# akshathmangudi/KAN-ViT

Measured on AMD Instinct MI355X. Metric: images/sec (train step) KAN-ViT 224x224, higher is better.
Workload: dtype f32

## Files before the change

kan-vit_amd/csrc/kan_bwd_weight_dma.hip:

```cpp
#include "kan_layer_common.h"

namespace {

typedef const __attribute__((address_space(1))) void* kvd_glb_ptr;
typedef __attribute__((address_space(3))) void* kvd_lds_ptr;

#ifndef KVD_NSLOT_N
#define KVD_NSLOT_N 4
#endif
constexpr int KVD_NSLOT = KVD_NSLOT_N;
constexpr int KVD_BLK = 16;
#ifndef KVD_ABLATE
#define KVD_ABLATE 0
#endif

template <int N>
__device__ __forceinline__ void kvd_wait_vm() {
    asm volatile("s_waitcnt vmcnt(%0)" ::"n"(N) : "memory");
}

template <int FAM, int GP, int NOT, bool BF>
__global__ __launch_bounds__(256) void kan_bwd_weight_dma_kernel(const LayerArgs a, int nfb, int nos, int tiles_per_bg, int shared,
                                                                 int nbg, int sub_rows, int cap, int placed) {
    constexpr int XF = KVD_BLK * 32;
    constexpr int YW = 32 * NOT;
    constexpr int SLOTF = XF + KVD_BLK * YW;
    constexpr int NDX = XF / 256;
    constexpr int NDY = KVD_BLK * YW / 256;
    constexpr int NDMA = NDX + NDY;
    static_assert(XF % 256 == 0 && (KVD_BLK * YW) % 256 == 0, "whole DMA instructions");
    static_assert(NDMA * (KVD_NSLOT - 1) < 64, "vmcnt is a 6-bit counter");
    extern __shared__ __attribute__((aligned(16))) float smem[];
    const int lane = threadIdx.x & 63, l31 = lane & 31, hf = lane >> 5;
    const int wave = __builtin_amdgcn_readfirstlane(threadIdx.x >> 6);
    const int gsz = nfb * nos;
    const int L = (int)(blockIdx.x & 7) * cap + (int)(blockIdx.x >> 3);
    int bg, slab, fb, os;
    if (placed) {
        const int set = L / gsz, mem = L - set * gsz;
        if (set >= nbg * a.msplit) return;
        bg = set % nbg, slab = set / nbg;
        fb = mem % nfb, os = mem / nfb;
    } else {
        const int units = gsz * nbg;
        if (L >= units * a.msplit) return;
        const int u = L % units;
// ... 33 lines not shown
    const char* dybase = reinterpret_cast<const char*>(a.dy + ms * a.ldy);
    int xrow[NDX], xcol[NDX], yrow[NDY], ycol[NDY];
#pragma unroll
    for (int k = 0; k < NDX; ++k) {
        const int c = 64 * k + lane;
        xrow[k] = c >> 3;
        xcol[k] = (c & 7) * 4;
    }
#pragma unroll
    for (int k = 0; k < NDY; ++k) {
        const int c = 64 * k + lane;
        const int row = c / (8 * NOT), rem = c - row * (8 * NOT), tile = rem >> 3;
        int tc = tcol[0];
#pragma unroll
        for (int i = 1; i < NOT; ++i) tc = tile == i ? tcol[i] : tc;
        yrow[k] = row;
        ycol[k] = tc + (rem & 7) * 4;
    }
    unsigned xo[NDX], yo[NDY];
#pragma unroll
    for (int k = 0; k < NDX; ++k) xo[k] = 4u * (unsigned)(xrow[k] * ldx32 + xcol[k]);
#pragma unroll
    for (int k = 0; k < NDY; ++k) yo[k] = 4u * (unsigned)(yrow[k] * ldy32 + ycol[k]);
    float* ring = smem + wave * (KVD_NSLOT * SLOTF);

    auto issue = [&](int blk, int slot) __attribute__((always_inline)) {
        if (KVD_ABLATE & 2) return;
        float* dst = ring + slot * SLOTF;
        const bool ragged = (blk + 1) * KVD_BLK > len;
        if (!ragged) {
            const char* xb = xbase + (long long)blk * (KVD_BLK * 4) * ldx32;
            const char* yb = dybase + (long long)blk * (KVD_BLK * 4) * ldy32;
#pragma unroll
            for (int k = 0; k < NDX; ++k) __builtin_amdgcn_global_load_lds((kvd_glb_ptr)(xb + xo[k]), (kvd_lds_ptr)(dst + 256 * k), 16, 0, 0);
#pragma unroll
            for (int k = 0; k < NDY; ++k) __builtin_amdgcn_global_load_lds((kvd_glb_ptr)(yb + yo[k]), (kvd_lds_ptr)(dst + XF + 256 * k), 16, 0, 0);
        } else {
#pragma unroll
            for (int k = 0; k < NDX; ++k) {
                int r = blk * KVD_BLK + xrow[k];
                r = r < len ? r : len - 1;
                __builtin_amdgcn_global_load_lds((kvd_glb_ptr)(xbase + 4u * (unsigned)(r * ldx32 + xcol[k])), (kvd_lds_ptr)(dst + 256 * k), 16, 0, 0);
            }
#pragma unroll
            for (int k = 0; k < NDY; ++k) {
                int r = blk * KVD_BLK + yrow[k];
                r = r < len ? r : len - 1;
                __builtin_amdgcn_global_load_lds((kvd_glb_ptr)(dybase + 4u * (unsigned)(r * ldy32 + ycol[k])), (kvd_lds_ptr)(dst + XF + 256 * k), 16, 0, 0);
            }
        }
    };

    constexpr int G0 = (FAM == KV_CHEBY && !BF) ? 1 : 0;
// ... 144 lines not shown
    __syncthreads();
    if (wave != 0) return;
    img = smem + lane;
    add();

    float* base = a.slab + (long long)slab * ((long long)a.groups * a.K * a.O);
#pragma unroll
    for (int i = 0; i < NOT; ++i) {
        if (tg[i] < 0) continue;
        const int tt = os * NOT + i;
        const int col0 = (tt % otpg) * 32;
        float* gb = base + (long long)tg[i] * a.K * a.O + col0 + l31;
#pragma unroll
        for (int j = 0; j < GP; ++j)
#pragma unroll
            for (int r = 0; r < 16; ++r) {
                const int fr = fb * 32 + kv_acc_row(r, hf);
                gb[((long long)fr * GP + j) * a.O] = j < G0 ? csum[i] : acc[j - G0][i][r];
            }
    }
}

template <int FAM, int GP, int NOT, bool BF>
int launch_dma(LayerArgs& a, const LayerBwdWeightPlan& pl, hipStream_t st) {
    const BwRegPlan& p = pl.r;
    const long long gsz = (long long)p.nfb * p.nos, sets = (long long)p.nbg * pl.slabs;
    const long long per_xcd = (sets * gsz + 7) / 8;
    const int placed = gsz <= 32 ? 1 : 0;
    const long long cap = placed ? (per_xcd + gsz - 1) / gsz * gsz : per_xcd;
    dim3 grid((unsigned)(8 * cap), 1, 1);
    constexpr size_t lds = sizeof(float) * 4 * KVD_NSLOT * (KVD_BLK * 32 * (1 + NOT));
    KV_ALLOW_LDS(160 * 1024, (kan_bwd_weight_dma_kernel<FAM, GP, NOT, BF>));
    hipLaunchKernelGGL((kan_bwd_weight_dma_kernel<FAM, GP, NOT, BF>), grid, dim3(256), lds, st, a, p.nfb, p.nos, p.tiles_per_bg, p.shared, p.nbg,
                       (int)(pl.rows_per_slab / 4), (int)cap, placed);
    KV_LAUNCH_CHECK("kan_bwd_weight_dma_kernel");
    return 0;
}

}

int kv_bwd_weight_dma(LayerArgs& a, const LayerBwdWeightPlan& p, hipStream_t st) {
    return p.bf ? launch_dma<KV_CHEBY, 5, 3, true>(a, p, st) : launch_dma<KV_CHEBY, 5, 3, false>(a, p, st);
}
```

kan-vit_amd/csrc/kan_bwd_weight_reg.hip:

```cpp
#include "kan_layer_common.h"

namespace {

template <int N, int I = 0, typename F>
__device__ __forceinline__ void kv_static_for(F&& f) {
    if constexpr (I < N) {
        f(std::integral_constant<int, I>{});
        kv_static_for<N, I + 1>(f);
    }
}

template <int FAM, int GP, int NOT, bool BF, int JC, bool PG, int ACT>
__device__ __forceinline__ void kan_bwd_weight_reg_kbody(const LayerArgs& a, int nfb, int nos, int tiles_per_bg, int shared, int nbg) {
    static_assert(!(PG && FAM == KV_RBF), "FastKAN's patch embedding reads u = LayerNorm(x): no gather form");
    static_assert(!(PG && BF), "the gather form is exact fp32 (bf16 MFMA phases are too short to hide the row walker: launch_bwd_weight_reg)");
    constexpr int NJC = (GP + JC - 1) / JC;
    constexpr bool RBF = (FAM == KV_RBF);
    constexpr int TS = BF ? 8 : 1;
    constexpr int UB = BF ? 1 : 4;
    constexpr int PD = BF ? (GP >= 28 ? 2 : 3) : 2;
    constexpr int NTOK = TS * UB;
    constexpr bool SCALAR_WAVE = FAM == KV_BSPLINE || FAM == KV_RBF || GP >= 28 || PG;
    const int lane = threadIdx.x & 63, l31 = lane & 31, hf = lane >> 5;
    const int wave = SCALAR_WAVE ? __builtin_amdgcn_readfirstlane(threadIdx.x >> 6) : (int)(threadIdx.x >> 6);
// ... 531 lines not shown
int kv_bwd_weight_reg(int family, LayerArgs& a, const LayerBwdWeightPlan& p, hipStream_t st) {
    if (p.form == LAYER_BWW_REG16) {
        if (family == KANVIT_RBF) return launch_bwd_weight_reg16<KV_RBF, 9, 9, 4>(a, p, st);
        return p.r.nt == 12 ? launch_bwd_weight_reg16<KV_BSPLINE, 9, 3, 12>(a, p, st) : launch_bwd_weight_reg16<KV_BSPLINE, 9, 3, 4>(a, p, st);
    }
    switch (family) {
        case KANVIT_LINEAR: return launch_bwd_weight_reg<KV_LINEAR, 1, 6>(a, p, st);
        case KANVIT_CHEBY: return p.r.nt == 1 ? launch_bwd_weight_reg<KV_CHEBY, 5, 1>(a, p, st) : launch_bwd_weight_reg<KV_CHEBY, 5, 3>(a, p, st);
        case KANVIT_BSPLINE:
            return p.r.nt == 3 ? launch_bwd_weight_reg<KV_BSPLINE, 9, 3, 5>(a, p, st) : launch_bwd_weight_reg<KV_BSPLINE, 9, 2, 5>(a, p, st);
        case KANVIT_RBF: return launch_bwd_weight_reg<KV_RBF, 9, 2>(a, p, st);
        case KANVIT_SINE:
            if (a.flags & KANVIT_FLAG_SINE_DFREQ) {
                if (a.GP == 28) return launch_bwd_weight_reg<KV_SINE_DF, 28, 4, 4>(a, p, st);
                return a.GP == 4 ? launch_bwd_weight_reg<KV_SINE_DF, 4, 2>(a, p, st) : launch_bwd_weight_reg<KV_SINE_DF, 5, 2>(a, p, st);
            }
            if (a.GP == 28) return launch_bwd_weight_reg<KV_SINE, 28, 4, 4>(a, p, st);
            return a.GP == 4 ? launch_bwd_weight_reg<KV_SINE, 4, 2>(a, p, st) : launch_bwd_weight_reg<KV_SINE, 5, 2>(a, p, st);
        case KANVIT_FOURIER: return launch_bwd_weight_reg<KV_FOURIER, 56, 4, 4>(a, p, st);
        default: return kv_fail(KANVIT_EINVAL, "unknown family %d", family);
    }
}

BwRegPlan plan_bwd_weight_reg(const kanvit_layer_desc* d) {
    BwRegPlan p{};
    if (kv_config().no_reg || kv_config().no_reg_bw) return p;
    p.njc = 1;
    p.gp = gp_of(d);
    const int fam = d->family;
    const RegBasis* rb = kv_reg_basis(d);
    if (!rb) return p;
    if (fam == KANVIT_BSPLINE && (d->flags & KANVIT_FLAG_BF16_MFMA) && !kv_config().no_bf16 && kv_config().bs_bw_bf16 == 1) return p;
    p.nt = rb->bww_nt;
    p.njc = rb->bww_njc;
    if (d->I % 32 || d->O % 32 || d->M < 256) return p;
    const int nshare = d->groups / d->x_group_mod;
    bool bf16_mode = (d->flags & KANVIT_FLAG_BF16_MFMA) && !kv_config().no_bf16;
    if (fam == KANVIT_BSPLINE && bf16_mode && kv_config().bs_bw_bf16 == 2) bf16_mode = false;
    p.bf = bf16_mode ? 1 : 0;
    if (((fam == KANVIT_BSPLINE && p.njc == 2) || fam == KANVIT_RBF) && !bf16_mode && !kv_config().bw_no_t16) {
        const int sh = (kv_share_ok(fam, d->flags) && nshare > 1) ? 1 : 0;
        const int t16 = (sh ? nshare : 1) * (d->O / 16);
        const int nc = (fam != KANVIT_RBF && t16 % 12 == 0) ? 12 : ((t16 % 4 == 0) ? 4 : 0);
        if (nc) {
            p.t16 = 1;
            p.shared = sh;
            p.nbg = sh ? d->x_group_mod : d->groups;
// ... 13 lines not shown
            if (S < 1) S = 1;
            if (S > 65535) return BwRegPlan{};
            long long rps = (d->M + S - 1) / S;
            rps = (rps + 15) / 16 * 16;
            p.rows_per_slab = rps;
            p.slabs = (int)((d->M + rps - 1) / rps);
            long long ld = d->ldx > d->ldy ? d->ldx : d->ldy;
            if (d->ldu > ld) ld = d->ldu;
            if (rps * ld + ld >= (1LL << 29) || units > (1LL << 30)) return BwRegPlan{};
            p.ok = true;
            return p;
        }
    }
    p.shared = (kv_share_ok(fam, d->flags) && nshare > 1) ? 1 : 0;
    p.nbg = p.shared ? d->x_group_mod : d->groups;
    p.tiles_per_bg = (p.shared ? nshare : 1) * (d->O / 32);
    p.nfb = d->I / 32;
    if (fam == KANVIT_BSPLINE && p.tiles_per_bg <= 2) p.nt = 2;
    p.nos = (p.tiles_per_bg + p.nt - 1) / p.nt;
    if (fam == KANVIT_CHEBY && p.nt == 3 && (long long)p.nbg * p.nfb * p.nos * (d->M / 64) < 4LL * N_CU && !kv_config().bw_dma_force) {
        p.nt = 1;
        p.nos = p.tiles_per_bg;
    }
    if (fam == KANVIT_CHEBY && p.nt == 3 && !kv_config().bw_no_dma && (bf16_mode || d->groups > 1) && d->ldx % 4 == 0 && d->ldy % 4 == 0) {
        const long long units = (long long)p.nbg * p.nfb * p.nos;
        long long r = 1;
        while ((long long)N_CU * r < units) ++r;
        long long S = (long long)N_CU * r / units;
        const bool force = kv_config().bw_dma_force != 0;
        const long long smax = force ? (d->M / 64 > 0 ? d->M / 64 : 1) : d->M / 256;
        if (S > smax) S = smax;
        if (S >= 1 && S <= 65535 && (force || units * S * 100 >= 85LL * N_CU * r)) {
            long long rps = (d->M + S - 1) / S;
            rps = (rps + 63) / 64 * 64;
            const long long ld = d->ldx > d->ldy ? d->ldx : d->ldy;
            if (rps / 4 * ld + ld < (1LL << 29) && units * S < (1LL << 31)) {
                p.dma = 1;
                p.rows_per_slab = rps;
                p.slabs = (int)((d->M + rps - 1) / rps);
                p.ok = true;
                return p;
            }
        }
    }
    const long long units = (long long)p.nbg * p.nfb * p.nos * p.njc;
    long long r = 1;
    while (4LL * N_CU * r < units) ++r;
    long long S = 4LL * N_CU * r / units;
    const long long smax = d->M / 64;
    if (S > smax) S = smax;
    if (S < 1) S = 1;
    if (S > 65535) S = 65535;
    const bool ln = fam == KANVIT_RBF && (d->flags & KANVIT_FLAG_FUSED_LN);
    if (ln && S * 4096 < d->M) S = (d->M + 4095) / 4096;
// ... 24 lines not shown
```

kan-vit_amd/csrc/kan_fwd_reg.hip:

```cpp
#include "kan_layer_common.h"

namespace {

template <int FAM, int NT, int NSH, int ICH, int GPC, int ACT>
__device__ __forceinline__ void kan_fwd_reg_body(const LayerArgs& a, float* __restrict__ smem, const int bx, const int by) {
    constexpr int BN = 32 * NT;
    constexpr int WROW = NSH * BN;
    constexpr int V4 = BN / 4;
    constexpr int IC = 2 * ICH;
    constexpr bool RBF = (FAM == KV_RBF);
    const int tid = threadIdx.x, lane = tid & 63, wave = tid >> 6, l31 = lane & 31, hf = lane >> 5;
    const int ntn = a.O / BN;
    const int gs = bx / ntn;
    const int n0 = (bx - gs * ntn) * BN;
    const int nsets = a.groups / NSH;
    const long long m0 = (long long)by * BM;
    constexpr int G0 = (FAM == KV_CHEBY && GPC > 0) ? 1 : 0;
    const int GP = GPC > 0 ? GPC : a.GP, GPE = GP - G0, KC = IC * GPE;
    const int nch = a.I / IC;
    const int WSZ = KC * WROW;
    const int mrem = (m0 + BM <= a.M) ? BM : (int)(a.M - m0);
    float* W_s = smem;

    const BasisArgs b = make_basis(a, gs);
// ... 238 lines not shown
            float* yp = a.y + yrow * a.ldy + (long long)g * a.O + col;
            const float* bp = a.bias ? a.bias + (long long)g * a.O + col : nullptr;
#pragma unroll
            for (int q = 0; q < 4; ++q) {
                f32x4 v = {acc[t][4 * q], acc[t][4 * q + 1], acc[t][4 * q + 2], acc[t][4 * q + 3]};
                if constexpr (G0 > 0) v += *reinterpret_cast<const f32x4*>(b_s + t * 32 + 8 * q + 4 * hf);
                if (bp) v += *reinterpret_cast<const f32x4*>(bp + 8 * q);
                if (posrow) v += *reinterpret_cast<const f32x4*>(posrow + col + 8 * q);
                *reinterpret_cast<f32x4*>(yp + 8 * q) = v;
                if (cls_owner) {
                    f32x4 cv = *reinterpret_cast<const f32x4*>(a.cls + col + 8 * q);
                    if (a.pos) cv += *reinterpret_cast<const f32x4*>(a.pos + col + 8 * q);
                    *reinterpret_cast<f32x4*>(yp - a.ldy + 8 * q) = cv;
                }
            }
        }
    }
}

template <int FAM, int NT, int NSH, int ICH, int GPC, bool TAIL, int ACT>
__device__ __forceinline__ void kan_fwd_reg_kbody(const LayerArgs& a) {
    extern __shared__ __attribute__((aligned(16))) float smem[];
    if constexpr (TAIL) {
        static_assert(NSH == 3, "the tail hands single projections of a shared-basis launch to the NSH = 1 body");
        const int ty = (int)blockIdx.y - a.tail_y0;
        if (ty >= 0) {
            const int tile = ty / 3, proj = ty - 3 * tile;
            kan_fwd_reg_body<FAM, NT, 1, ICH, GPC, ACT>(a, smem, proj * (int)gridDim.x + (int)blockIdx.x, a.tail_y0 + tile);
            return;
        }
    }
    kan_fwd_reg_body<FAM, NT, NSH, ICH, GPC, ACT>(a, smem, (int)blockIdx.x, (int)blockIdx.y);
}
template <int FAM, int NT, int NSH, int ICH, int GPC = 0, bool TAIL = false>
__global__ __launch_bounds__(256, GPC ? 2 : 1) void kan_fwd_reg_kernel(const LayerArgs a) {
    kan_fwd_reg_kbody<FAM, NT, NSH, ICH, GPC, TAIL, KV_ACT_SILU>(a);
}
template <int FAM, int NT, int NSH, int ICH, int GPC = 0, bool TAIL = false>
__global__ __launch_bounds__(256, GPC ? 2 : 1) void kan_fwd_reg_act_kernel(const LayerArgs a) {
    kan_fwd_reg_kbody<FAM, NT, NSH, ICH, GPC, TAIL, KV_ACT_DYN>(a);
}

template <int FAM, int NT, int NSH, int ICH, int GPC = 0>
int launch_fwd_reg(const LayerArgs& a, const LayerFwdPlan& p, hipStream_t st) {
    const dim3 grid(p.gx, p.gy, 1);
    if constexpr (NSH == 3 && GPC > 0) {
        if (p.tail_y0 != 0x7fffffff) {
            KV_ACT_ALLOW_LDS(FAM, a.base_act, 160 * 1024, kan_fwd_reg_kernel, kan_fwd_reg_act_kernel, (FAM, NT, NSH, ICH, GPC, true));
            KV_ACT_LAUNCH(FAM, a.base_act, kan_fwd_reg_kernel, kan_fwd_reg_act_kernel, (FAM, NT, NSH, ICH, GPC, true), grid, dim3(256), p.lds, st, a);
            KV_LAUNCH_CHECK("kan_fwd_reg_kernel");
            return 0;
        }
    }
    KV_ACT_ALLOW_LDS(FAM, a.base_act, 160 * 1024, kan_fwd_reg_kernel, kan_fwd_reg_act_kernel, (FAM, NT, NSH, ICH, GPC));
    KV_ACT_LAUNCH(FAM, a.base_act, kan_fwd_reg_kernel, kan_fwd_reg_act_kernel, (FAM, NT, NSH, ICH, GPC), grid, dim3(256), p.lds, st, a);
    KV_LAUNCH_CHECK("kan_fwd_reg_kernel");
    return 0;
}

template <int FAM, int NT, int NSH>
int launch_fwd_reg_ich(const LayerArgs& a, const LayerFwdPlan& p, hipStream_t st) {
    if (p.gpc && p.ich == 4) {
        if constexpr (FAM == KV_LINEAR) return launch_fwd_reg<FAM, NT, NSH, 4, 1>(a, p, st);
        if constexpr (FAM == KV_CHEBY) return launch_fwd_reg<FAM, NT, NSH, 4, 5>(a, p, st);
        if constexpr (FAM == KV_BSPLINE || FAM == KV_RBF) return launch_fwd_reg<FAM, NT, NSH, 4, 9>(a, p, st);
        if constexpr (FAM == KV_SINE) return launch_fwd_reg<FAM, NT, NSH, 4, 4>(a, p, st);
    }
    if (p.gpc && p.ich == 2) {
        if constexpr (FAM == KV_BSPLINE || FAM == KV_RBF) return launch_fwd_reg<FAM, NT, NSH, 2, 9>(a, p, st);
// ... 32 lines not shown
```

kan-vit_amd/csrc/kan_layer.hip:

```cpp
#include "kan_layer_common.h"

extern "C" int kanvit_layer_ln_fusable(const kanvit_layer_desc* d);

namespace {

int validate(const kanvit_layer_desc* d, const char* who) {
    if (!d) return kv_fail(KANVIT_EINVAL, "%s: null descriptor", who);
    const int gp = gp_of(d);
    if (gp < 1) return kv_fail(KANVIT_EINVAL, "%s: unknown family %d or G=%d", who, d->family, d->G);
    if (gp > 80) return kv_fail(KANVIT_EINVAL, "%s: %d generated columns per feature exceeds the supported 80", who, gp);
    if (d->groups < 1 || d->x_group_mod < 1 || d->groups % d->x_group_mod != 0)
        return kv_fail(KANVIT_EINVAL, "%s: groups=%d must be a positive multiple of x_group_mod=%d", who, d->groups,
                       d->x_group_mod);
    if (d->groups > 65535) return kv_fail(KANVIT_EINVAL, "%s: groups=%d exceeds 65535", who, d->groups);
    if ((d->M + BM - 1) / BM > 65535) return kv_fail(KANVIT_EINVAL, "%s: M=%lld exceeds %d rows per launch", who,
                                                     (long long)d->M, 65535 * BM);
    if (d->I < 1 || d->O < 1 || d->M < 0) return kv_fail(KANVIT_EINVAL, "%s: bad sizes M=%lld I=%d O=%d", who,
                                                          (long long)d->M, d->I, d->O);
    if ((long long)d->I * gp > 0x7fffffffLL / 4) return kv_fail(KANVIT_EINVAL, "%s: K too large", who);
    if (d->ldx < (int64_t)d->x_group_mod * d->I) return kv_fail(KANVIT_EINVAL, "%s: ldx=%lld < x_group_mod*I", who,
                                                                 (long long)d->ldx);
    if (d->ldy < (int64_t)d->groups * d->O) return kv_fail(KANVIT_EINVAL, "%s: ldy=%lld < groups*O", who,
                                                            (long long)d->ldy);
    if (d->family == KANVIT_BSPLINE) {
        const int nk = d->G + d->spline_order + 1;
        if (d->spline_order < 0 || d->G < 1 || nk > KV_MAX_KNOTS)
            return kv_fail(KANVIT_EINVAL, "%s: bspline G=%d order=%d unsupported (knots %d > %d)", who, d->G,
// ... 84 lines not shown
    if (fam == KANVIT_SINE && ((al.bp & 15) || (d->bparam_stride & 3))) return;
    const long long ldx = pd ? d->I : d->ldx;
    const bool has_u = fam == KANVIT_RBF && al.has_u && !is_ln(d);
    const int wrow = 32 * nt * nsh, wrs = 256 / (8 * nt);
    const RegBasis* rb = kv_config().no_pipe ? nullptr : kv_reg_basis(d);
    for (int ich = 4; ich >= 1; ich >>= 1) {
        const int ic = 2 * ich, kc = ic * gp;
        if (d->I % ic) continue;
        if (pd && (((pd->W / pd->n_patches) % ic) || (ich == 4 && (pd->W & 3)))) continue;
        if (ich == 4 && ((ldx & 3) || (d->I & 3) || (al.x & 15) || (has_u && ((d->ldu & 3) || (al.u & 15))))) continue;
        if ((kc + wrs - 1) / wrs > (share3 ? 4 : 8)) continue;
        if ((long long)kc * d->O >= (1LL << 30)) continue;
        size_t lds = sizeof(float) * 2 * (size_t)kc * wrow;
        if (lds < sizeof(float) * 4 * 32 * 36) lds = sizeof(float) * 4 * 32 * 36;
        if (lds > 160 * 1024) continue;
        p.form = LAYER_FWD_REG;
        p.nt = nt;
        p.nsh = nsh;
        p.ich = ich;
        p.gpc = rb ? rb->fwd_gpc[ich == 4 ? 0 : (ich == 2 ? 1 : 2)] : 0;
        p.lds = lds;
        p.gx = (unsigned)((d->groups / nsh) * (d->O / (32 * nt)));
        p.gy = (unsigned)tiles;
        if (nsh == 3 && p.gpc > 0) {
            const int t1 = kv_tail_first_tile(tiles, (int)p.gx);
            if (t1 < tiles) {
                p.tail_y0 = t1;
                p.gy = (unsigned)(t1 + 3 * (tiles - t1));
            }
        }
        return;
    }
}

void plan_fwd_reg_bf16_form(const kanvit_layer_desc* d, const kanvit_patch_desc* pd, LayerFwdPlan& p) {
    const FwdRegBf16Plan& r = p.rb;
    p.nt = r.nt;
    p.nsh = r.nsh;
    p.ich = r.ich;
    p.ws_bytes = r.ws_bytes;
    p.gx = (unsigned)((d->groups / r.nsh) * (d->O / (32 * r.nt)));
    p.gy = (unsigned)((d->M + BM - 1) / BM);
    p.lds = r.lds;
    p.form = pd ? LAYER_FWD_REG_BF16_PATCH : LAYER_FWD_REG_BF16;
    if (pd || r.ich != 8 || !(d->family == KANVIT_LINEAR || d->family == KANVIT_CHEBY)) return;
    const size_t wlds = (size_t)r.nch * r.vs * 2 * 32 * r.nt * r.nsh * 16 + sizeof(float) * 32 * r.nt * r.nsh;
    if (wlds > 150 * 1024 || r.nch != 4 || d->M < 4096 || p.gx > N_CU || kv_config().no_ws) return;
    const long long ntiles = (d->M + KV_WS_THREADS / 2 - 1) / (KV_WS_THREADS / 2);
    long long py = N_CU / p.gx;
    if (py > ntiles) py = ntiles;
    if (py < 1) py = 1;
// ... 147 lines not shown
                p.nci = d->I / ic;
                p.lds = sizeof(float) * (2 * 16 * ws2 + (fam == KANVIT_SINE ? (size_t)nshare * 4 * gp : 0));
                if (fam != KANVIT_SINE && p.nci > 1) p.tail_y0 = kv_tail_first_tile(tiles, d->x_group_mod);
                const long long t1 = p.tail_y0 < tiles ? p.tail_y0 : tiles;
                p.gy = (unsigned)(t1 + p.nci * (tiles - t1));
                return p;
            }
        }
        if (is_ln(d)) return plan_none(p, "kanvit_layer_bwd_input: KANVIT_FLAG_FUSED_LN needs the register kernel (alignment / shape)");
        p.form = LAYER_BWI_TILE;
        p.ic = kv_tile_bwd_input_ic(fam, d->I, gp, d->G, nshare, 0);
        if (!p.ic) return plan_none(p, "kanvit_layer_bwd_input: tile does not fit the LDS");
    }
    p.kt = (p.ic * gp + 31) / 32;
    p.nci = (d->I + p.ic - 1) / p.ic;
    p.lds = kv_tile_bwd_input_lds(fam, p.ic, gp, d->G, nshare, p.form == LAYER_BWI_TILE_BF16 ? d->O : 0);
    return p;
}

static const char* const KV_PATCH_BWW_UNCOVERED =
    "kanvit_patch_embed_bwd_weight: layer / geometry not covered by the gathering weight-gradient kernels "
    "(kanvit_patch_embed_bwd_weight_ok); use patchify + kanvit_layer_bwd_weight";

LayerBwdWeightPlan plan_layer_bwd_weight(const kanvit_layer_desc* d, const kanvit_patch_desc* pd, const LayerAlign& al) {
    LayerBwdWeightPlan p{};
    p.total = (long long)d->groups * d->I * gp_of(d) * d->O;
    auto slabs = [&p](int ws_slabs, int n, long long rows) {
        p.slabs = n;
        p.rows_per_slab = rows;
        p.ws_bytes = ws_slabs > 1 ? sizeof(float) * (size_t)ws_slabs * (size_t)p.total : 0;
    };
    if (kv_tiny_ok(d)) {
        if (pd) return plan_none(p, KV_PATCH_BWW_UNCOVERED);
        const int s = (int)((d->M + 127) / 128 < 64 ? (d->M + 127) / 128 : 64);
        const long long rows = ((d->M + s - 1) / s + 63) / 64 * 64;
        slabs(s, (int)((d->M + rows - 1) / rows), rows);
        p.form = LAYER_BWW_TINY;
        return p;
    }
    p.r = plan_bwd_weight_reg(d);
    if (p.r.ok) {
        slabs(p.r.slabs, p.r.slabs, p.r.rows_per_slab);
        p.bf = p.r.bf;
        if (pd) {
            if (d->groups != 1 || p.r.bf || p.r.t16 || !kv_reg_basis(d)->bww_pg) return plan_none(p, KV_PATCH_BWW_UNCOVERED);
            p.form = LAYER_BWW_REG_PATCH;
        } else if (p.r.t16) {
            p.form = LAYER_BWW_REG16;
        } else {
            p.form = (p.r.dma && !((al.x | al.dy) & 15)) ? LAYER_BWW_DMA : LAYER_BWW_REG;
        }
        return p;
    }
    if (pd) return plan_none(p, KV_PATCH_BWW_UNCOVERED);
    p.t = plan_bwd_weight(d);
    slabs(p.t.msplit, p.t.msplit, p.t.rows_per_split);
    p.bf = ((d->flags & KANVIT_FLAG_BF16_MFMA) && !kv_config().no_bf16) ? 1 : 0;
    if (is_ln(d)) return plan_none(p, "kanvit_layer_bwd_weight: KANVIT_FLAG_FUSED_LN needs the register kernel (shape)");
    if ((long long)BW_ROWS * d->ldy >= (1LL << 30)) return plan_none(p, "kanvit_layer_bwd_weight: ldy too large for 32-bit tile offsets");
    const int kt = (p.t.ic * gp_of(d) + 31) / 32;
    p.lds = sizeof(float) * 2 * ((size_t)BW_ROWS * (p.t.ic | 1) * (d->family == KANVIT_RBF ? 2 : 1) + (size_t)BW_ROWS * 32 * BW_NT * p.t.nsh +
                                 (size_t)kt * 32 * BW_AS);
    if (p.lds > 160 * 1024) return plan_none(p, "kanvit_layer_bwd_weight: tile does not fit the LDS");
    p.form = p.bf ? LAYER_BWW_TILE_BF16 : LAYER_BWW_TILE;
    return p;
}

static KvTinyArgs tiny_args(const kanvit_layer_desc* d) {
    KvTinyArgs t{};
// ... 181 lines not shown
    patch_args(a, p, cls, pos);
    const LayerFwdPlan pl = plan_layer_fwd(d, p, layer_align(images, nullptr, w, bparams ? bparams : w, bias ? bias : w, y, nullptr, nullptr, nullptr));
    return launch_layer_fwd(d, a, pl, "kanvit_patch_embed_fwd", workspace, workspace_bytes, (hipStream_t)stream);
}

int kanvit_patch_embed_fwd(const kanvit_layer_desc* d, const kanvit_patch_desc* p, const float* images, const float* w,
                           const float* bparams, const float* bias, const float* cls, const float* pos, float* y, void* stream) {
    if (d && (d->flags & KANVIT_FLAG_BF16_MFMA) && !kv_config().no_bf16)
        return kv_fail(KANVIT_EINVAL, "kanvit_patch_embed_fwd: KANVIT_FLAG_BF16_MFMA needs a workspace (kanvit_patch_embed_fwd_ws)");
    return kanvit_patch_embed_fwd_ws(d, p, images, w, bparams, bias, cls, pos, y, nullptr, 0, stream);
}

static bool patch_bwd_weight_geometry_ok(const kanvit_layer_desc* d, const kanvit_patch_desc* p) {
    if (!desc_ok(d) || !p || d->groups != 1 || d->x_group_mod != 1 || d->M < 1) return false;
    if (p->C < 1 || p->H < 1 || p->W < 1 || p->n_patches < 1 || p->H % p->n_patches || p->W % p->n_patches) return false;
    if (p->prepend_rows != 0 && p->prepend_rows != 1) return false;
    const long long P = (long long)p->n_patches * p->n_patches;
    if (d->I != (long long)p->C * (p->H / p->n_patches) * (p->W / p->n_patches) || d->M % P) return false;
    const long long B = d->M / P;
    return B * p->C * p->H * p->W < (1LL << 31) && (d->M + B * p->prepend_rows + 1) * d->ldy < (1LL << 31);
}

int kanvit_patch_embed_bwd_weight_ok(const kanvit_layer_desc* d, const kanvit_patch_desc* p) {
    return patch_bwd_weight_geometry_ok(d, p) && plan_layer_bwd_weight(d, p, LayerAlign{}).form == LAYER_BWW_REG_PATCH;
}

size_t kanvit_patch_embed_bwd_weight_workspace(const kanvit_layer_desc* d, const kanvit_patch_desc* p) {
    if (!patch_bwd_weight_geometry_ok(d, p)) return 0;
    const LayerBwdWeightPlan pl = plan_layer_bwd_weight(d, p, LayerAlign{});
    return pl.form == LAYER_BWW_REG_PATCH ? pl.ws_bytes : 0;
}

static int launch_layer_bwd_weight(const kanvit_layer_desc* d, LayerArgs& a, const LayerBwdWeightPlan& p, float* dw, void* workspace,
                                   hipStream_t st) {
    if (p.form == LAYER_BWW_NONE) return kv_fail(KANVIT_EINVAL, p.why, p.why_a, p.why_b);
    a.rows_per_split = p.rows_per_slab;
    a.msplit = p.slabs;
    a.slab = p.slabs > 1 ? (float*)workspace : dw;
    int rc;
    switch (p.form) {
        case LAYER_BWW_TINY: {
            KvTinyArgs t = tiny_args(d);
            t.x = a.x; t.bp = a.bp; t.dy = a.dy;
            t.slabs = p.slabs; t.rows_per_slab = p.rows_per_slab; t.slab = a.slab;
            rc = kv_tiny_bwd_weight(t, st);
            break;
        }
        case LAYER_BWW_DMA: rc = kv_bwd_weight_dma(a, p, st); break;
        case LAYER_BWW_REG16:
        case LAYER_BWW_REG:
        case LAYER_BWW_REG_PATCH: rc = kv_bwd_weight_reg(d->family, a, p, st); break;
        default:
            a.IC = p.t.ic;
            a.nchunks_n = p.t.nchunks_n;
            rc = kv_tile_bwd_weight(d->family, a, p, st);
    }
    if (rc || p.slabs <= 1) return rc;
    return kv_slab_reduce((const float*)workspace, dw, p.total, p.slabs, st);
}

int kanvit_patch_embed_bwd_weight(const kanvit_layer_desc* d, const kanvit_patch_desc* p, const float* images, const float* bparams,
                                  const float* dy, float* dw, void* workspace, size_t workspace_bytes, void* stream) {
    if (int rc = validate(d, "kanvit_patch_embed_bwd_weight")) return rc;
    if (int rc = patch_validate(d, p, "kanvit_patch_embed_bwd_weight")) return rc;
    if (!dw) return kv_fail(KANVIT_EINVAL, "kanvit_patch_embed_bwd_weight: null dw");
    if (d->M == 0) {
        KV_HIP_CHECK(hipMemsetAsync(dw, 0, sizeof(float) * (size_t)d->I * gp_of(d) * d->O, (hipStream_t)stream));
        return 0;
    }
    if (!images || !dy) return kv_fail(KANVIT_EINVAL, "kanvit_patch_embed_bwd_weight: null images/dy");
    if (needs_bparams(d->family) && !bparams) return kv_fail(KANVIT_EINVAL, "kanvit_patch_embed_bwd_weight: family %d needs bparams", d->family);
    const LayerBwdWeightPlan pl = plan_layer_bwd_weight(d, p, layer_align(images, nullptr, nullptr, nullptr, nullptr, nullptr, dy, nullptr, nullptr));
    if ((d->flags & KANVIT_FLAG_SINE_DFREQ) && !pl.r.ok)
        return kv_fail(KANVIT_EINVAL, "kanvit_patch_embed_bwd_weight: KANVIT_FLAG_SINE_DFREQ is not available for this layer (kanvit_layer_sine_dfreq_ok)");
    if (!patch_bwd_weight_geometry_ok(d, p) || pl.form != LAYER_BWW_REG_PATCH) return kv_fail(KANVIT_EINVAL, KV_PATCH_BWW_UNCOVERED);
    if (pl.ws_bytes > 0 && (!workspace || workspace_bytes < pl.ws_bytes))
        return kv_fail(KANVIT_ENOMEM, "kanvit_patch_embed_bwd_weight: workspace %zu bytes < required %zu", workspace_bytes, pl.ws_bytes);
    LayerArgs a = base_args(d);
    a.x = images;
    a.bp = bparams;
    a.dy = dy;
    patch_args(a, p, nullptr, nullptr);
    return launch_layer_bwd_weight(d, a, pl, dw, workspace, (hipStream_t)stream);
}

int kanvit_layer_sine_dfreq_ok(const kanvit_layer_desc* d) {
    if (!desc_ok(d) || d->family != KANVIT_SINE || d->M < 1) return 0;
    return plan_layer_bwd_weight(d, nullptr, LayerAlign{}).r.ok ? 1 : 0;
}

int64_t kanvit_layer_dparam_tiles(const kanvit_layer_desc* d) {
    if (!d || d->family != KANVIT_SINE) return 0;
    return (d->M + BM - 1) / BM;
}

size_t kanvit_layer_bwd_input_workspace(const kanvit_layer_desc* d) {
    if (!desc_ok(d)) return 0;
    return plan_layer_bwd_input(d, LayerAlign{}).ws_max;
// ... 140 lines not shown
```

kan-vit_amd/csrc/kan_layer_common.h:

```cpp
#pragma once
#include "kan_basis.h"

#include <type_traits>
#include "kanvit_common.h"

#include <stdlib.h>

constexpr int BM = 128;
constexpr int NTHR = 512;
constexpr int NPROD = 256;
constexpr int AS = BM + 1;
constexpr int BIN_NC = 32;
constexpr int BW_ROWS = 32;
constexpr int BW_AS = BW_ROWS + 1;
constexpr int BW_NT = 2;
constexpr int BW_TPW = 5;
constexpr int BW_KC_MAX = 288;
constexpr int N_CU = 256;

struct LayerArgs {
    const float* x;
    const float* u;
    const float* w;
    const float* bp;
// ... 16 lines not shown
    int vcols;
    int ln;
    float ln_eps;
    float* stats;
    int tail_y0;
    int base_act;
    int vec;
};
constexpr int KV_VEC_W = 1, KV_VEC_DY = 2;

inline int kv_tail_first_tile(long long tiles, int per_tile) {
    const int cfg = kv_config().tail;
    if (cfg == 0 || tiles < 2) return (int)tiles;
    if (cfg > 0) return (int)(tiles - (cfg < tiles ? cfg : tiles - 1));
    const long long wgs = tiles * per_tile;
    const long long per_cu = wgs / N_CU;
    if (per_cu < 4) return (int)tiles;
    const long long rest = wgs - per_cu * N_CU + N_CU / 4;
    long long t1 = (wgs - rest) / per_tile;
    if (t1 < tiles / 2) t1 = tiles / 2;
    return (int)t1;
}

__device__ __forceinline__ BasisArgs make_basis(const LayerArgs& a, int g) {
    BasisArgs b;
    b.G = a.G;
    b.GP = a.GP;
    b.order = a.order;
    b.nk = a.nk;
    b.has_base = a.has_base;
    b.inv_h = a.rbf_inv_h;
    b.bp = a.bp ? a.bp + (long long)g * a.bp_stride : nullptr;
    b.uniform = (a.flags & KANVIT_FLAG_UNIFORM_KNOTS) && a.order == 3;
    b.act = a.base_act;
    return b;
}

template <int ICH>
__device__ __forceinline__ void kv_ln_row_stats(const float* __restrict__ xh, int nch, int I, float eps, float& mean, float& rstd) {
    float s = 0.0f;
    for (int c = 0; c < nch; ++c)
#pragma unroll
        for (int e = 0; e < ICH; ++e) s += xh[c * 2 * ICH + e];
    s += __shfl_xor(s, 32);
    mean = s / (float)I;
    float q = 0.0f;
// ... 141 lines not shown
    int gp, kt, fph, nci;
    int vcols;
    size_t lds, ws_bytes;
};

struct BwPlan {
    int ic, nfchunks, nchunks_n, msplit, nsh;
    long long rows_per_split;
};

struct BwRegPlan {
    bool ok;
    int gp, nt, nfb, nos, tiles_per_bg, nbg, shared, slabs, njc;
    int t16;
    int bf;
    int dma;
    long long rows_per_slab;
};

enum LayerFwdForm { LAYER_FWD_NONE, LAYER_FWD_TINY, LAYER_FWD_WS_BF16, LAYER_FWD_REG_BF16, LAYER_FWD_REG_BF16_PATCH, LAYER_FWD_TILE_BF16,
                    LAYER_FWD_REG, LAYER_FWD_TILE };
enum LayerBwdInputForm { LAYER_BWI_NONE, LAYER_BWI_TINY, LAYER_BWI_RES_BF16, LAYER_BWI_REG_BF16, LAYER_BWI_REG_BF16_WIDE, LAYER_BWI_TILE_BF16,
                         LAYER_BWI_REG, LAYER_BWI_TILE };
enum LayerBwdWeightForm { LAYER_BWW_NONE, LAYER_BWW_TINY, LAYER_BWW_DMA, LAYER_BWW_REG16, LAYER_BWW_REG, LAYER_BWW_REG_PATCH, LAYER_BWW_TILE,
                          LAYER_BWW_TILE_BF16 };

struct LayerAlign {
    uintptr_t x, u, w, bp, bias, y, dy, dx, du;
    int has_u;
    int vec() const { return ((w & 15) ? 0 : KV_VEC_W) | ((dy & 15) ? 0 : KV_VEC_DY); }
};

struct LayerFwdPlan {
    LayerFwdForm form;
    const char* why;
    int why_a, why_b;
    int nt, nsh;
    int ich, gpc;
    int ic, fast;
    int strip;
    int tail_y0;
    unsigned gx, gy;
    size_t lds;
    size_t ws_bytes;
    size_t ws_max;
    FwdRegBf16Plan rb;
    FwdBf16Plan tb;
// ... 49 lines not shown
    return sizeof(float) * ((size_t)BM * (ic | 1) * (family == KANVIT_RBF ? 8 : 4) + (family == KANVIT_SINE ? (size_t)nshare * 4 * G : 0) +
                            (size_t)kct * AS + 2 * ops);
}

inline int kv_tile_bwd_input_ic(int family, int I, int gp, int G, int nshare, int bf_O) {
    int ic = 96 / gp;
    if (ic < 1) ic = 1;
    if (ic > I) ic = I;
    while (ic > 1 && kv_tile_bwd_input_lds(family, ic, gp, G, nshare, bf_O) > 160 * 1024) --ic;
    return kv_tile_bwd_input_lds(family, ic, gp, G, nshare, bf_O) > 160 * 1024 ? 0 : ic;
}

int kv_fwd_reg(int family, const LayerArgs& a, const LayerFwdPlan& p, hipStream_t st);
int kv_fwd_reg_bf16(int family, LayerArgs& a, const LayerFwdPlan& p, void* ws, hipStream_t st);
int kv_tile_fwd(int family, LayerArgs& a, const LayerFwdPlan& p, hipStream_t st);
int kv_tile_fwd_bf16(int family, LayerArgs& a, const LayerFwdPlan& p, void* ws, hipStream_t st);
int kv_bwd_input_reg(int family, const LayerArgs& a, const LayerBwdInputPlan& p, hipStream_t st);
int kv_bwd_input_reg_bf16(int family, LayerArgs& a, const LayerBwdInputPlan& p, hipStream_t st);
int kv_tile_bwd_input(int family, LayerArgs& a, const LayerBwdInputPlan& p, hipStream_t st);
FwdRegBf16Plan plan_fwd_reg_bf16(const kanvit_layer_desc* d);
FwdBf16Plan plan_fwd_bf16(const kanvit_layer_desc* d);
BwdRegBf16Plan plan_bwd_input_reg_bf16(const kanvit_layer_desc* d);
BwPlan plan_bwd_weight(const kanvit_layer_desc* d);
BwRegPlan plan_bwd_weight_reg(const kanvit_layer_desc* d);
int kv_tile_bwd_weight(int family, const LayerArgs& a, const LayerBwdWeightPlan& p, hipStream_t st);
int kv_bwd_weight_reg(int family, LayerArgs& a, const LayerBwdWeightPlan& p, hipStream_t st);
int kv_bwd_weight_dma(LayerArgs& a, const LayerBwdWeightPlan& p, hipStream_t st);
int kv_slab_reduce(const float* slab, float* dw, long long total, int slabs, hipStream_t st);
```

Baseline: 1621.

## Add DMA gather form for patch-embed weight gradient and split wide forward tail

Adds a patch-gathering variant of the DMA weight-gradient kernel. Each lane walks patch offsets incrementally and the per-row offsets are broadcast with ds_bpermute, so global_load_lds can read image pixels directly instead of going through the register-path patch kernel. The planner now enables DMA for fp32 single-group patch layers, tries a few extra rounds to reach the occupancy threshold, and selects the new form when x and dy are aligned. It also extends the forward tail splitting to single-shared-basis Chebyshev launches by cutting wide column tiles into pieces. This adds complexity and bpermute overhead per issue, and the tail split can add more small blocks.

Result: no change. 1624, median of 6 (+0.2%).

```diff
diff --git a/kan-vit_amd/csrc/kan_bwd_weight_dma.hip b/kan-vit_amd/csrc/kan_bwd_weight_dma.hip
--- a/kan-vit_amd/csrc/kan_bwd_weight_dma.hip
+++ b/kan-vit_amd/csrc/kan_bwd_weight_dma.hip
@@ -19,9 +19,46 @@
     asm volatile("s_waitcnt vmcnt(%0)" ::"n"(N) : "memory");
 }
 
-template <int FAM, int GP, int NOT, bool BF>
-__global__ __launch_bounds__(256) void kan_bwd_weight_dma_kernel(const LayerArgs a, int nfb, int nos, int tiles_per_bg, int shared,
-                                                                 int nbg, int sub_rows, int cap, int placed) {
+struct PatchJump {
+    int px, py;
+    unsigned xoff, dyoff;
+    int n, r, q;
+    unsigned dx0, dy0, line_wrap, img_wrap, pre_ldy;
+    __device__ __forceinline__ void init(const LayerArgs& a, long long m_) {
+        n = a.pg_n;
+        const int P = n * n, ph = a.pg_H / n, pw = a.pg_W / n;
+        const int m = (int)(m_ < a.M ? m_ : a.M - 1);
+        const int smp = m / P, pidx = m - smp * P;
+        py = pidx / n;
+        px = pidx - py * n;
+        xoff = (unsigned)((smp * a.pg_C * a.pg_H + py * ph) * a.pg_W + px * pw);
+        const unsigned ldy = (unsigned)a.ldy;
+        pre_ldy = (unsigned)a.pg_pre * ldy;
+        dyoff = (unsigned)(m + (smp + 1) * a.pg_pre) * ldy;
+        const int s = KVD_BLK / P, rem = KVD_BLK - s * P;
+        q = rem / n;
+        r = rem - q * n;
+        line_wrap = (unsigned)(ph * a.pg_W - n * pw);
+        img_wrap = (unsigned)((a.pg_C * a.pg_H - n * ph) * a.pg_W);
+        dx0 = (unsigned)(r * pw + q * ph * a.pg_W + s * a.pg_C * a.pg_H * a.pg_W);
+        dy0 = (unsigned)KVD_BLK * ldy + (unsigned)s * pre_ldy;
+    }
+    __device__ __forceinline__ void jump() {
+        px += r;
+        const bool w1 = px >= n;
+        px -= w1 ? n : 0;
+        py += q + (w1 ? 1 : 0);
+        const bool w2 = py >= n;
+        py -= w2 ? n : 0;
+        xoff += dx0 + (w1 ? line_wrap : 0u) + (w2 ? img_wrap : 0u);
+        dyoff += dy0 + (w2 ? pre_ldy : 0u);
+    }
+};
+
+template <int FAM, int GP, int NOT, bool BF, bool PG>
+__device__ __forceinline__ void kan_bwd_weight_dma_body(const LayerArgs& a, int nfb, int nos, int tiles_per_bg, int shared,
+                                                        int nbg, int sub_rows, int cap, int placed) {
+    static_assert(!(PG && BF), "the gather form is exact fp32");
     constexpr int XF = KVD_BLK * 32;
     constexpr int YW = 32 * NOT;
     constexpr int SLOTF = XF + KVD_BLK * YW;
@@ -101,13 +138,35 @@
     for (int k = 0; k < NDX; ++k) xo[k] = 4u * (unsigned)(xrow[k] * ldx32 + xcol[k]);
 #pragma unroll
     for (int k = 0; k < NDY; ++k) yo[k] = 4u * (unsigned)(yrow[k] * ldy32 + ycol[k]);
+    PatchJump walk;
+    unsigned pg_f[NDX];
+    if constexpr (PG) {
+        walk.init(a, ms + (lane & (KVD_BLK - 1)));
+#pragma unroll
+        for (int k = 0; k < NDX; ++k) pg_f[k] = (unsigned)kv_patch_feature_offset(a, fb * 32 + xcol[k]);
+    }
     float* ring = smem + wave * (KVD_NSLOT * SLOTF);
 
     auto issue = [&](int blk, int slot) __attribute__((always_inline)) {
         if (KVD_ABLATE & 2) return;
         float* dst = ring + slot * SLOTF;
         const bool ragged = (blk + 1) * KVD_BLK > len;
-        if (!ragged) {
+        if constexpr (PG) {
+            const int last = len - 1 - blk * KVD_BLK;
+#pragma unroll
+            for (int k = 0; k < NDX; ++k) {
+                const int r = xrow[k] < last ? xrow[k] : last;
+                const unsigned o = (unsigned)__builtin_amdgcn_ds_bpermute(r << 2, (int)walk.xoff) + pg_f[k];
+                __builtin_amdgcn_global_load_lds((kvd_glb_ptr)(a.x + o), (kvd_lds_ptr)(dst + 256 * k), 16, 0, 0);
+            }
+#pragma unroll
+            for (int k = 0; k < NDY; ++k) {
+                const int r = yrow[k] < last ? yrow[k] : last;
+                const unsigned o = (unsigned)__builtin_amdgcn_ds_bpermute(r << 2, (int)walk.dyoff) + (unsigned)ycol[k];
+                __builtin_amdgcn_global_load_lds((kvd_glb_ptr)(a.dy + o), (kvd_lds_ptr)(dst + XF + 256 * k), 16, 0, 0);
+            }
+            walk.jump();
+        } else if (!ragged) {
             const char* xb = xbase + (long long)blk * (KVD_BLK * 4) * ldx32;
             const char* yb = dybase + (long long)blk * (KVD_BLK * 4) * ldy32;
 #pragma unroll
@@ -298,6 +357,17 @@
 }
 
 template <int FAM, int GP, int NOT, bool BF>
+__global__ __launch_bounds__(256) void kan_bwd_weight_dma_kernel(const LayerArgs a, int nfb, int nos, int tiles_per_bg, int shared,
+                                                                 int nbg, int sub_rows, int cap, int placed) {
+    kan_bwd_weight_dma_body<FAM, GP, NOT, BF, false>(a, nfb, nos, tiles_per_bg, shared, nbg, sub_rows, cap, placed);
+}
+template <int FAM, int GP, int NOT>
+__global__ __launch_bounds__(256) void kan_bwd_weight_dma_patch_kernel(const LayerArgs a, int nfb, int nos, int tiles_per_bg, int shared,
+                                                                       int nbg, int sub_rows, int cap, int placed) {
+    kan_bwd_weight_dma_body<FAM, GP, NOT, false, true>(a, nfb, nos, tiles_per_bg, shared, nbg, sub_rows, cap, placed);
+}
+
+template <int FAM, int GP, int NOT, bool BF, bool PG = false>
 int launch_dma(LayerArgs& a, const LayerBwdWeightPlan& pl, hipStream_t st) {
     const BwRegPlan& p = pl.r;
     const long long gsz = (long long)p.nfb * p.nos, sets = (long long)p.nbg * pl.slabs;
@@ -306,15 +376,23 @@
     const long long cap = placed ? (per_xcd + gsz - 1) / gsz * gsz : per_xcd;
     dim3 grid((unsigned)(8 * cap), 1, 1);
     constexpr size_t lds = sizeof(float) * 4 * KVD_NSLOT * (KVD_BLK * 32 * (1 + NOT));
-    KV_ALLOW_LDS(160 * 1024, (kan_bwd_weight_dma_kernel<FAM, GP, NOT, BF>));
-    hipLaunchKernelGGL((kan_bwd_weight_dma_kernel<FAM, GP, NOT, BF>), grid, dim3(256), lds, st, a, p.nfb, p.nos, p.tiles_per_bg, p.shared, p.nbg,
-                       (int)(pl.rows_per_slab / 4), (int)cap, placed);
-    KV_LAUNCH_CHECK("kan_bwd_weight_dma_kernel");
+    if constexpr (PG) {
+        KV_ALLOW_LDS(160 * 1024, (kan_bwd_weight_dma_patch_kernel<FAM, GP, NOT>));
+        hipLaunchKernelGGL((kan_bwd_weight_dma_patch_kernel<FAM, GP, NOT>), grid, dim3(256), lds, st, a, p.nfb, p.nos, p.tiles_per_bg, p.shared,
+                           p.nbg, (int)(pl.rows_per_slab / 4), (int)cap, placed);
+        KV_LAUNCH_CHECK("kan_bwd_weight_dma_patch_kernel");
+    } else {
+        KV_ALLOW_LDS(160 * 1024, (kan_bwd_weight_dma_kernel<FAM, GP, NOT, BF>));
+        hipLaunchKernelGGL((kan_bwd_weight_dma_kernel<FAM, GP, NOT, BF>), grid, dim3(256), lds, st, a, p.nfb, p.nos, p.tiles_per_bg, p.shared, p.nbg,
+                           (int)(pl.rows_per_slab / 4), (int)cap, placed);
+        KV_LAUNCH_CHECK("kan_bwd_weight_dma_kernel");
+    }
     return 0;
 }
 
 }
 
 int kv_bwd_weight_dma(LayerArgs& a, const LayerBwdWeightPlan& p, hipStream_t st) {
+    if (p.form == LAYER_BWW_DMA_PATCH) return launch_dma<KV_CHEBY, 5, 3, false, true>(a, p, st);
     return p.bf ? launch_dma<KV_CHEBY, 5, 3, true>(a, p, st) : launch_dma<KV_CHEBY, 5, 3, false>(a, p, st);
 }
diff --git a/kan-vit_amd/csrc/kan_bwd_weight_reg.hip b/kan-vit_amd/csrc/kan_bwd_weight_reg.hip
--- a/kan-vit_amd/csrc/kan_bwd_weight_reg.hip
+++ b/kan-vit_amd/csrc/kan_bwd_weight_reg.hip
@@ -577,7 +577,7 @@
     }
 }
 
-BwRegPlan plan_bwd_weight_reg(const kanvit_layer_desc* d) {
+BwRegPlan plan_bwd_weight_reg(const kanvit_layer_desc* d, const kanvit_patch_desc* pd) {
     BwRegPlan p{};
     if (kv_config().no_reg || kv_config().no_reg_bw) return p;
     p.njc = 1;
@@ -637,14 +637,20 @@
         p.nt = 1;
         p.nos = p.tiles_per_bg;
     }
-    if (fam == KANVIT_CHEBY && p.nt == 3 && !kv_config().bw_no_dma && (bf16_mode || d->groups > 1) && d->ldx % 4 == 0 && d->ldy % 4 == 0) {
+    const bool gather = pd && !bf16_mode && d->groups == 1 && pd->n_patches > 0 && (pd->W / pd->n_patches) % 4 == 0;
+    if (fam == KANVIT_CHEBY && p.nt == 3 && !kv_config().bw_no_dma && (bf16_mode || d->groups > 1 || gather) && d->ldx % 4 == 0 && d->ldy % 4 == 0) {
         const long long units = (long long)p.nbg * p.nfb * p.nos;
         long long r = 1;
         while ((long long)N_CU * r < units) ++r;
-        long long S = (long long)N_CU * r / units;
         const bool force = kv_config().bw_dma_force != 0;
         const long long smax = force ? (d->M / 64 > 0 ? d->M / 64 : 1) : d->M / 256;
+        long long S = (long long)N_CU * r / units;
         if (S > smax) S = smax;
+        for (int more = gather && !force ? 3 : 0; more > 0 && units * S * 100 < 85LL * N_CU * r; --more) {
+            ++r;
+            S = (long long)N_CU * r / units;
+            if (S > smax) S = smax;
+        }
         if (S >= 1 && S <= 65535 && (force || units * S * 100 >= 85LL * N_CU * r)) {
             long long rps = (d->M + S - 1) / S;
             rps = (rps + 63) / 64 * 64;
diff --git a/kan-vit_amd/csrc/kan_fwd_reg.hip b/kan-vit_amd/csrc/kan_fwd_reg.hip
--- a/kan-vit_amd/csrc/kan_fwd_reg.hip
+++ b/kan-vit_amd/csrc/kan_fwd_reg.hip
@@ -284,11 +284,17 @@
 __device__ __forceinline__ void kan_fwd_reg_kbody(const LayerArgs& a) {
     extern __shared__ __attribute__((aligned(16))) float smem[];
     if constexpr (TAIL) {
-        static_assert(NSH == 3, "the tail hands single projections of a shared-basis launch to the NSH = 1 body");
+        static_assert(NSH == 3 || (NSH == 1 && NT > kv_fwd_tail_nt(NT)), "the tail cuts a shared-basis launch into projections, a wide one into column pieces");
         const int ty = (int)blockIdx.y - a.tail_y0;
         if (ty >= 0) {
-            const int tile = ty / 3, proj = ty - 3 * tile;
-            kan_fwd_reg_body<FAM, NT, 1, ICH, GPC, ACT>(a, smem, proj * (int)gridDim.x + (int)blockIdx.x, a.tail_y0 + tile);
+            if constexpr (NSH == 3) {
+                const int tile = ty / 3, proj = ty - 3 * tile;
+                kan_fwd_reg_body<FAM, NT, 1, ICH, GPC, ACT>(a, smem, proj * (int)gridDim.x + (int)blockIdx.x, a.tail_y0 + tile);
+            } else {
+                constexpr int PNT = kv_fwd_tail_nt(NT), NP = NT / PNT;
+                const int tile = ty / NP, piece = ty - NP * tile;
+                kan_fwd_reg_body<FAM, PNT, 1, ICH, GPC, ACT>(a, smem, (int)blockIdx.x * NP + piece, a.tail_y0 + tile);
+            }
             return;
         }
     }
@@ -306,7 +312,7 @@
 template <int FAM, int NT, int NSH, int ICH, int GPC = 0>
 int launch_fwd_reg(const LayerArgs& a, const LayerFwdPlan& p, hipStream_t st) {
     const dim3 grid(p.gx, p.gy, 1);
-    if constexpr (NSH == 3 && GPC > 0) {
+    if constexpr (kv_fwd_tail_pieces(FAM, NT, NSH, GPC) > 1) {
         if (p.tail_y0 != 0x7fffffff) {
             KV_ACT_ALLOW_LDS(FAM, a.base_act, 160 * 1024, kan_fwd_reg_kernel, kan_fwd_reg_act_kernel, (FAM, NT, NSH, ICH, GPC, true));
             KV_ACT_LAUNCH(FAM, a.base_act, kan_fwd_reg_kernel, kan_fwd_reg_act_kernel, (FAM, NT, NSH, ICH, GPC, true), grid, dim3(256), p.lds, st, a);
diff --git a/kan-vit_amd/csrc/kan_layer.hip b/kan-vit_amd/csrc/kan_layer.hip
--- a/kan-vit_amd/csrc/kan_layer.hip
+++ b/kan-vit_amd/csrc/kan_layer.hip
@@ -3,6 +3,8 @@
 extern "C" int kanvit_layer_ln_fusable(const kanvit_layer_desc* d);
 
 namespace {
+
+static_assert(KV_CHEBY == KANVIT_CHEBY, "kv_fwd_tail_pieces is asked with the descriptor's family");
 
 int validate(const kanvit_layer_desc* d, const char* who) {
     if (!d) return kv_fail(KANVIT_EINVAL, "%s: null descriptor", who);
@@ -133,11 +135,11 @@
         p.lds = lds;
         p.gx = (unsigned)((d->groups / nsh) * (d->O / (32 * nt)));
         p.gy = (unsigned)tiles;
-        if (nsh == 3 && p.gpc > 0) {
+        if (const int np = kv_fwd_tail_pieces(fam, nt, nsh, p.gpc); np > 1) {
             const int t1 = kv_tail_first_tile(tiles, (int)p.gx);
-            if (t1 < tiles) {
+            if (t1 < tiles && t1 + np * (tiles - t1) <= 65535) {
                 p.tail_y0 = t1;
-                p.gy = (unsigned)(t1 + 3 * (tiles - t1));
+                p.gy = (unsigned)(t1 + np * (tiles - t1));
             }
         }
         return;
@@ -331,6 +333,8 @@
     "kanvit_patch_embed_bwd_weight: layer / geometry not covered by the gathering weight-gradient kernels "
     "(kanvit_patch_embed_bwd_weight_ok); use patchify + kanvit_layer_bwd_weight";
 
+static bool kv_bww_gathers(LayerBwdWeightForm f) { return f == LAYER_BWW_REG_PATCH || f == LAYER_BWW_DMA_PATCH; }
+
 LayerBwdWeightPlan plan_layer_bwd_weight(const kanvit_layer_desc* d, const kanvit_patch_desc* pd, const LayerAlign& al) {
     LayerBwdWeightPlan p{};
     p.total = (long long)d->groups * d->I * gp_of(d) * d->O;
@@ -347,13 +351,13 @@
         p.form = LAYER_BWW_TINY;
         return p;
     }
-    p.r = plan_bwd_weight_reg(d);
+    p.r = plan_bwd_weight_reg(d, pd);
     if (p.r.ok) {
         slabs(p.r.slabs, p.r.slabs, p.r.rows_per_slab);
         p.bf = p.r.bf;
         if (pd) {
             if (d->groups != 1 || p.r.bf || p.r.t16 || !kv_reg_basis(d)->bww_pg) return plan_none(p, KV_PATCH_BWW_UNCOVERED);
-            p.form = LAYER_BWW_REG_PATCH;
+            p.form = (p.r.dma && !((al.x | al.dy) & 15)) ? LAYER_BWW_DMA_PATCH : LAYER_BWW_REG_PATCH;
         } else if (p.r.t16) {
             p.form = LAYER_BWW_REG16;
         } else {
@@ -581,13 +585,13 @@
 }
 
 int kanvit_patch_embed_bwd_weight_ok(const kanvit_layer_desc* d, const kanvit_patch_desc* p) {
-    return patch_bwd_weight_geometry_ok(d, p) && plan_layer_bwd_weight(d, p, LayerAlign{}).form == LAYER_BWW_REG_PATCH;
+    return patch_bwd_weight_geometry_ok(d, p) && kv_bww_gathers(plan_layer_bwd_weight(d, p, LayerAlign{}).form);
 }
 
 size_t kanvit_patch_embed_bwd_weight_workspace(const kanvit_layer_desc* d, const kanvit_patch_desc* p) {
     if (!patch_bwd_weight_geometry_ok(d, p)) return 0;
     const LayerBwdWeightPlan pl = plan_layer_bwd_weight(d, p, LayerAlign{});
-    return pl.form == LAYER_BWW_REG_PATCH ? pl.ws_bytes : 0;
+    return kv_bww_gathers(pl.form) ? pl.ws_bytes : 0;
 }
 
 static int launch_layer_bwd_weight(const kanvit_layer_desc* d, LayerArgs& a, const LayerBwdWeightPlan& p, float* dw, void* workspace,
@@ -605,7 +609,8 @@
             rc = kv_tiny_bwd_weight(t, st);
             break;
         }
-        case LAYER_BWW_DMA: rc = kv_bwd_weight_dma(a, p, st); break;
+        case LAYER_BWW_DMA:
+        case LAYER_BWW_DMA_PATCH: rc = kv_bwd_weight_dma(a, p, st); break;
         case LAYER_BWW_REG16:
         case LAYER_BWW_REG:
         case LAYER_BWW_REG_PATCH: rc = kv_bwd_weight_reg(d->family, a, p, st); break;
@@ -632,7 +637,7 @@
     const LayerBwdWeightPlan pl = plan_layer_bwd_weight(d, p, layer_align(images, nullptr, nullptr, nullptr, nullptr, nullptr, dy, nullptr, nullptr));
     if ((d->flags & KANVIT_FLAG_SINE_DFREQ) && !pl.r.ok)
         return kv_fail(KANVIT_EINVAL, "kanvit_patch_embed_bwd_weight: KANVIT_FLAG_SINE_DFREQ is not available for this layer (kanvit_layer_sine_dfreq_ok)");
-    if (!patch_bwd_weight_geometry_ok(d, p) || pl.form != LAYER_BWW_REG_PATCH) return kv_fail(KANVIT_EINVAL, KV_PATCH_BWW_UNCOVERED);
+    if (!patch_bwd_weight_geometry_ok(d, p) || !kv_bww_gathers(pl.form)) return kv_fail(KANVIT_EINVAL, KV_PATCH_BWW_UNCOVERED);
     if (pl.ws_bytes > 0 && (!workspace || workspace_bytes < pl.ws_bytes))
         return kv_fail(KANVIT_ENOMEM, "kanvit_patch_embed_bwd_weight: workspace %zu bytes < required %zu", workspace_bytes, pl.ws_bytes);
     LayerArgs a = base_args(d);
diff --git a/kan-vit_amd/csrc/kan_layer_common.h b/kan-vit_amd/csrc/kan_layer_common.h
--- a/kan-vit_amd/csrc/kan_layer_common.h
+++ b/kan-vit_amd/csrc/kan_layer_common.h
@@ -62,6 +62,13 @@
     return (int)t1;
 }
 
+constexpr int kv_fwd_tail_nt(int) { return 1; }
+constexpr int kv_fwd_tail_pieces(int family, int nt, int nsh, int gpc) {
+    if (gpc <= 0) return 1;
+    if (nsh == 3) return 3;
+    return (nsh == 1 && nt > 1 && family == KV_CHEBY) ? nt / kv_fwd_tail_nt(nt) : 1;
+}
+
 __device__ __forceinline__ BasisArgs make_basis(const LayerArgs& a, int g) {
     BasisArgs b;
     b.G = a.G;
@@ -249,7 +256,7 @@
                     LAYER_FWD_REG, LAYER_FWD_TILE };
 enum LayerBwdInputForm { LAYER_BWI_NONE, LAYER_BWI_TINY, LAYER_BWI_RES_BF16, LAYER_BWI_REG_BF16, LAYER_BWI_REG_BF16_WIDE, LAYER_BWI_TILE_BF16,
                          LAYER_BWI_REG, LAYER_BWI_TILE };
-enum LayerBwdWeightForm { LAYER_BWW_NONE, LAYER_BWW_TINY, LAYER_BWW_DMA, LAYER_BWW_REG16, LAYER_BWW_REG, LAYER_BWW_REG_PATCH, LAYER_BWW_TILE,
+enum LayerBwdWeightForm { LAYER_BWW_NONE, LAYER_BWW_TINY, LAYER_BWW_DMA, LAYER_BWW_REG16, LAYER_BWW_REG, LAYER_BWW_REG_PATCH, LAYER_BWW_DMA_PATCH, LAYER_BWW_TILE,
                           LAYER_BWW_TILE_BF16 };
 
 struct LayerAlign {
@@ -345,7 +352,7 @@
 FwdBf16Plan plan_fwd_bf16(const kanvit_layer_desc* d);
 BwdRegBf16Plan plan_bwd_input_reg_bf16(const kanvit_layer_desc* d);
 BwPlan plan_bwd_weight(const kanvit_layer_desc* d);
-BwRegPlan plan_bwd_weight_reg(const kanvit_layer_desc* d);
+BwRegPlan plan_bwd_weight_reg(const kanvit_layer_desc* d, const kanvit_patch_desc* pd = nullptr);
 int kv_tile_bwd_weight(int family, const LayerArgs& a, const LayerBwdWeightPlan& p, hipStream_t st);
 int kv_bwd_weight_reg(int family, LayerArgs& a, const LayerBwdWeightPlan& p, hipStream_t st);
 int kv_bwd_weight_dma(LayerArgs& a, const LayerBwdWeightPlan& p, hipStream_t st);
```
